# xiaoxubeii/kubernetes-schedule-simulator

Measured on AMD Instinct MI355X. Metric: pods scheduled/sec + node-evals/sec at 100k nodes, 1/2/4/8 MI355X, higher is better.
Workload: dtype int64; 1 GPU; C3: 100000 nodes, 1000000-pod queue, default predicates + LeastRequested(1) + BalancedResourceAllocation(1); nodes=100000, global_batch=35715, mode=persistent, blocks=256, parallelism=single-gpu

## Files before the change

include/ksim.h:

```cpp
#ifndef KSIM_H
#define KSIM_H

#include <stdint.h>

#ifdef __cplusplus
extern "C" {
#endif

#define KSIM_ABI_VERSION 7

#define KSIM_OK 0
#define KSIM_E_INVAL (-1)
#define KSIM_E_DEVICE (-2)
#define KSIM_E_NOMEM (-3)
#define KSIM_E_UNSUPPORTED (-4)
#define KSIM_E_STATE (-5)
#define KSIM_E_OVERFLOW (-6)
#define KSIM_E_NO_NODES (-7)

#define KSIM_MAX_SCALAR 8
#define KSIM_MAX_RCLASS 16
#define KSIM_MAX_WIDE 256
#define KSIM_NREASONS 32
#define KSIM_MAX_RANKS 8
// ... 351 lines not shown
  int64_t n_nodes;
  int32_t max_vols[3];
  int32_t zone_words;
  const uint32_t* key_filter;
  const int32_t* vc;
  const uint32_t* vc_filter;
  const ksim_vol_ref* refs;
  const uint32_t* zone_ok;
  const uint64_t* slots;
  const int32_t* slot_count;
} ksim_volume_tables;

int ksim_load_volumes(ksim_handle* h, const ksim_volume_tables* t);
int ksim_grow_volumes(ksim_handle* h, const ksim_volume_tables* t);
int ksim_read_volumes(ksim_handle* h, uint64_t* slots, int32_t* slot_count);

int ksim_read_nodes(ksim_handle* h, ksim_node_state* out);
int ksim_get_counter(ksim_handle* h, uint64_t* out);
int ksim_set_counter(ksim_handle* h, uint64_t value);

#define KSIM_FORM_FAST 1
#define KSIM_FORM_STREAM 2
#define KSIM_FORM_CACHED 4
#define KSIM_FORM_ROWS_SHIFT 8
int ksim_last_form(ksim_handle* h, int32_t* form);

int ksim_selftest(void);

#ifdef __cplusplus
}
#endif
#endif
```

kubernetes-schedule-simulator_amd/csrc/ksim_handle.h:

```cpp
#pragma once
#include <hip/hip_runtime.h>

#include <algorithm>
#include <atomic>
#include <array>
#include <cstdarg>
#include <cstdio>
#include <cstdlib>
#include <cstring>
#include <map>
#include <string>
#include <vector>

#include "ksim_common.h"
#include "ksim_pgen.h"
#include "ksim_sweep.h"
#include "ksim_tree.h"
#include "ksim_f64.h"

extern "C" hipError_t ksim_launch_scan(const KsimCtx* c, int npt, int collect, int grid, hipStream_t s);
extern "C" hipError_t ksim_launch_eval(const KsimCtx* c, int64_t pod, uint8_t* fit, uint32_t* reasons, int64_t* score,
                                       uint8_t* rcls, hipStream_t s);
extern "C" int ksim_scan_coresident(int npt, int collect, int grid);
extern "C" int ksim_one_npt(int64_t n);
// ... 4 lines not shown
extern "C" hipError_t ksim_launch_serve(const KsimCtx* c, const KsimServeArgs* a, int npt, int grid, int aux, hipStream_t s);
extern "C" hipError_t ksim_launch_ipa_pass(const KsimCtx* c, int npt, int grid, hipStream_t s);
extern "C" hipError_t ksim_launch_assume(const KsimCtx* c, int64_t pod, int64_t node, int32_t* status, hipStream_t s);
extern "C" hipError_t ksim_launch_persistent(const KsimCtx* c, const KsimCtx* cdev, uint64_t* granules, int grid,
                                             int lds_rows, hipStream_t s);
extern "C" int ksim_persistent_config(int64_t n, int* grid, int* lds_rows);
extern "C" size_t ksim_persistent_granule_bytes(int grid);
extern "C" hipError_t ksim_sweep_prepare(const int64_t* ac, const int64_t* am, int64_t n, double* dac, double* dam,
                                         double* yc, double* ym, hipStream_t st);
extern "C" hipError_t ksim_sweep_launch(const int64_t* rc0, const int64_t* rm0, const int64_t* zc0, const int64_t* zm0,
                                        const int32_t* c0, const ksim_pod* pods, void* fpods, const SwArgsWhy* args,
                                        int32_t n_scen, const uint32_t* absent, int32_t absent_words, hipEvent_t ev0,
                                        hipEvent_t ev1, hipStream_t st);
extern "C" hipError_t ksim_sweep_general_launch(const KsimCtx* hc, const SwgCols* cols, const SwgArgsPre* args,
                                                const SwgSpread* spr, const SwgAffinity* ipa, const SwgVolumes* vol,
                                                int32_t n_scen, const uint32_t* absent, int32_t absent_words,
                                                int32_t* err, hipEvent_t ev0, hipEvent_t ev1, hipStream_t st);
extern "C" int ksim_pfast_config(int64_t n, int max_grid, int stream, int* grid, int* lds_rows);
extern "C" hipError_t ksim_pstream_prepare(const KsimCtx* c, double* mirror, hipStream_t s);
extern "C" size_t ksim_pfast_granule_bytes(void);
extern "C" size_t ksim_shard_xchg_bytes(void);
extern "C" size_t ksim_shard_lx_offset(void);
extern "C" size_t ksim_pfast_cache_bytes(int lds_rows, int ncls);
extern "C" int ksim_pfast_rows_per_thread(int lds_rows, int stream);
extern "C" hipError_t ksim_launch_pfast(const KsimCtx* c, uint64_t* granules, int grid, int lds_rows, double* mirror,
                                        const KsimShard* sh, const int32_t* tcls, const KsimTreeClass* tclass, int ncls,
                                        hipStream_t s);
extern "C" hipError_t ksim_tree_build(const KsimCtx* c, const KsimTreeGeo* g, const KsimTreeClass* cls,
                                      const int32_t* tcls, int32_t* leaves, uint64_t* levels, int32_t* fitc,
                                      double* ty, const KsimTreeSweep* sw, hipStream_t s);
extern "C" hipError_t ksim_tree_build_absent(const KsimCtx* c, const KsimTreeGeo* g, const KsimTreeClass* cls,
                                             const int32_t* tcls, int32_t* leaves, uint64_t* levels, int32_t* fitc,
                                             double* ty, const KsimTreeSweep* sw, hipStream_t s);
extern "C" hipError_t ksim_tree_sweep_init(const KsimCtx* c, const KsimTreeSweep* sw, hipStream_t s);
extern "C" hipError_t ksim_tree_sweep_absent(const KsimCtx* c, const KsimTreeSweep* sw, const uint32_t* absent,
                                             int32_t words, hipStream_t s);
extern "C" hipError_t ksim_tree_launch(const KsimCtx* c, const KsimTreeGeo* g, const KsimTreeClass* cls,
                                       const int32_t* tcls, int32_t* leaves, uint64_t* levels, int32_t* fitc,
                                       double* ty, const KsimTreeSweep* sw, hipStream_t s);
struct KsimRelayout;
extern "C" hipError_t ksim_launch_relayout(const KsimRelayout* r, hipStream_t s);
extern "C" hipError_t ksim_launch_set_row(const KsimCtx* c, int64_t node, const uint64_t* pack, int32_t full,
                                          hipStream_t s);
extern "C" hipError_t ksim_launch_release(const KsimCtx* c, int64_t pod, int64_t node, hipStream_t s);
extern "C" hipError_t ksim_launch_undo(const KsimCtx* c, const KsimTentRec* t, hipStream_t s);
extern "C" hipError_t ksim_launch_remap_hosts(ksim_pod* pods, int64_t n_pods, int64_t idx, int32_t op, hipStream_t s);
extern "C" hipError_t ksim_launch_pod_k(ksim_pod* pods, int64_t n_pods, const KsimCtx* c, hipStream_t s);
extern "C" hipError_t ksim_launch_port_max(const int32_t* port_count, int64_t n, int32_t* out, hipStream_t s);

struct DevBuf {
// ... 257 lines not shown
```

kubernetes-schedule-simulator_amd/csrc/ksim_pfast.hip:

```cpp
#include <algorithm>

#include "ksim_decide.h"
#include "ksim_f64.h"
#include "ksim_fast.h"
#include "ksim_tree.h"
#include "ksim_wave.h"
#include "ksim_xchg.h"

using namespace kf64;

namespace {

#ifndef KSIM_PF_BS
#define KSIM_PF_BS 512
#endif
constexpr int BS = KSIM_PF_BS;
constexpr int NW = BS / 64;
constexpr int RW = NW - 1;
constexpr int RT = RW * 64;
constexpr int MAXB = 4;
constexpr int MAXG = 64 * MAXB;
constexpr int NSLOT = 4;
constexpr int FIXSTRIDE = 16;
constexpr int RING = 16;
constexpr int RING_FILL = 8;
constexpr uint64_t SPIN_LIMIT_TICKS = 200000000ull;
constexpr int ANSLOT = 8;
// ... 82 lines not shown
  int32_t rank, world;
  int64_t node_base;
  uint32_t xtag_base;
  uint64_t* xchg;
  uint64_t* peers[KSIM_MAX_RANKS];
  uint64_t start_ticks;
  double* mirror;
  const int32_t* tcls;
  const KsimTreeClass* tclass;
  int32_t ncls;
};

namespace {

struct FRows {
  double *ac, *am, *rc, *rm, *zc, *zm, *yc, *ym;
  int32_t *allowed, *count;
  uint32_t* fl;
  int32_t* ev;
  int32_t* ev2;
  uint32_t* rm2;
  uint32_t* rma;
  int16_t* cache;
};

constexpr int LDS_ROW_BYTES = 8 * 8 + 8 * 4;
constexpr int LDS_ROW_BYTES_STREAM = 7 * 4;

extern __shared__ __attribute__((aligned(16))) char kf_smem[];

template <bool STREAM>
__device__ __forceinline__ FRows carve(int rows, const PfArgs& a, int64_t lo) {
  FRows r;
  if (STREAM) {
    double* m = a.mirror + lo;
    const int64_t n = a.n;
    r.ac = m; r.am = m + n; r.rc = m + 2 * n; r.rm = m + 3 * n;
    r.zc = m + 4 * n; r.zm = m + 5 * n; r.yc = nullptr; r.ym = nullptr;
    r.allowed = const_cast<int32_t*>(a.allowed_pods) + lo;
    r.count = a.pod_count + lo;
    r.fl = const_cast<uint32_t*>(a.flags) + lo;
    int32_t* q = reinterpret_cast<int32_t*>(kf_smem);
    r.ev = q;
    r.ev2 = q + 2 * rows;
    r.rm2 = reinterpret_cast<uint32_t*>(q + 3 * rows);
    r.rma = r.rm2 + 2 * rows;
    r.cache = nullptr;
    return r;
  }
  double* d = reinterpret_cast<double*>(kf_smem);
  r.ac = d; r.am = d + rows; r.rc = d + 2 * rows; r.rm = d + 3 * rows;
  r.zc = d + 4 * rows; r.zm = d + 5 * rows; r.yc = d + 6 * rows; r.ym = d + 7 * rows;
  int32_t* q = reinterpret_cast<int32_t*>(d + 8 * rows);
  r.allowed = q; r.count = q + rows;
  r.fl = reinterpret_cast<uint32_t*>(q + 2 * rows);
  r.ev = q + 3 * rows;
  r.ev2 = q + 5 * rows;
  r.rm2 = reinterpret_cast<uint32_t*>(q + 6 * rows);
  r.cache = reinterpret_cast<int16_t*>(q + 8 * rows);
  return r;
}

typedef __attribute__((address_space(1))) const uint64_t cgu64;
typedef __attribute__((address_space(1))) const int32_t cgi32;
__device__ __forceinline__ double ld_l2(const double* p) {
  return __builtin_bit_cast(double, __hip_atomic_load((cgu64*)p, __ATOMIC_RELAXED, __HIP_MEMORY_SCOPE_AGENT));
}
__device__ __forceinline__ int32_t ld_l2(const int32_t* p) {
  return __hip_atomic_load((cgi32*)p, __ATOMIC_RELAXED, __HIP_MEMORY_SCOPE_AGENT);
}
__device__ __forceinline__ FRow load_frow_l2(const FRows& R, int32_t j) {
  FRow r;
  r.ac = ld_l2(R.ac + j); r.am = ld_l2(R.am + j); r.rc = ld_l2(R.rc + j); r.rm = ld_l2(R.rm + j);
  r.zc = ld_l2(R.zc + j); r.zm = ld_l2(R.zm + j);
  r.yc = r.ac != 0.0 ? 1.0 / r.ac : 0.0;
  r.ym = r.am != 0.0 ? 1.0 / r.am : 0.0;
  r.allowed = ld_l2(R.allowed + j); r.count = ld_l2(R.count + j);
  r.fl = (uint32_t)ld_l2(reinterpret_cast<const int32_t*>(R.fl) + j);
  return r;
}

template <bool STREAM>
__device__ __forceinline__ FRow load_frow(const FRows& R, int32_t j) {
  FRow r;
  r.ac = R.ac[j]; r.am = R.am[j]; r.rc = R.rc[j]; r.rm = R.rm[j]; r.zc = R.zc[j]; r.zm = R.zm[j];
  if (STREAM) {
    r.yc = r.ac != 0.0 ? 1.0 / r.ac : 0.0;
    r.ym = r.am != 0.0 ? 1.0 / r.am : 0.0;
  } else {
    r.yc = R.yc[j]; r.ym = R.ym[j];
  }
  r.allowed = R.allowed[j]; r.count = R.count[j]; r.fl = R.fl[j];
  return r;
}

struct Top2 {
  int32_t f, m1, c1, m2, c2;
};

}

template <int NPT, bool STREAM, bool CACHE>
__global__ __launch_bounds__(BS) void ksim_pfast_kernel(PfArgs a) {
  static_assert(!(STREAM && CACHE), "the cached form keeps the rows in LDS");
  __shared__ int32_t s_wst[2][RW][5];
  __shared__ uint64_t s_bm[2][NPT][RW];
  __shared__ int32_t s_wg[2][5];
  __shared__ int32_t s_fix[2][2];
  __shared__ int32_t s_hist[KSIM_NREASONS];
  __shared__ int32_t s_mode[2], s_own[2];
  __shared__ int32_t s_arr;
  __shared__ int32_t s_prow[2];
  __shared__ double s_pdel[2][4];
  __shared__ double s_pval[4];
  __shared__ int32_t s_pcnt;
  __shared__ __attribute__((aligned(16))) ksim_pod s_pod[RING];
  __shared__ int32_t s_pcls[CACHE ? RING : 1];
  __shared__ KsimTreeClass s_tcl[CACHE ? KSIM_TREE_MAX_CLASSES : 1];
#ifdef KSIM_STAMPS
  uint64_t st_acc[16] = {};
#endif

  const int tid = threadIdx.x, lane = tid & 63, wv = tid >> 6;
  const int rt = tid - 64;
  const int G = gridDim.x;
  const int me = blockIdx.x;
  const int64_t chunk = a.chunk;
  const int64_t lo = (int64_t)me * chunk;
// ... 28 lines not shown
    if (p < a.end) reinterpret_cast<uint4*>(&s_pod[p % RING])[lane % 8] = v;
    if (CACHE && lane < RING_FILL && p0 + lane < a.end) s_pcls[(p0 + lane) % RING] = cl;
  };
  uint4 ring_next = make_uint4(0, 0, 0, 0);
  int32_t ring_next_cl = 0;
  if (wv == 1) {
    uint4 v;
    int32_t cl = 0;
    ring_load(a.first, v, cl);
    ring_load(a.first + RING_FILL, ring_next, ring_next_cl);
    ring_store(a.first, v, cl);
  }
  if (CACHE)
    for (int k = tid; k < a.ncls; k += BS) s_tcl[k] = a.tclass[k];
  if (tid == 0) { s_fix[a.first & 1][0] = -1; s_arr = 0; s_prow[0] = s_prow[1] = -1; }
  uint64_t counter = *a.counter;
  __syncthreads();
  auto cls_fpod = [&](int k) -> FPod {
    const KsimTreeClass& t = s_tcl[k];
    return FPod{t.rq_c, t.rq_m, t.nz_c, t.nz_m, 0.0, 0.0, t.anyreq, t.be};
  };
  if (CACHE) {
    const int tot = a.ncls * nrows;
    for (int idx = tid; idx < tot; idx += BS) {
      const int k = idx / nrows, j = idx - k * nrows;
      uint32_t rm;
      R.cache[k * chunk + j] = (int16_t)feval(EC, cls_fpod(k), load_frow<false>(R, j), rm);
    }
    __syncthreads();
  }

  auto ptag = [&](int64_t p) -> uint64_t { return (uint64_t)((p - a.first + 1) & 0xFF); };
  auto wave_stats = [&](const int32_t (&e)[NPT], int buf, int w) {
    int32_t v = -1, nf = 0;
#pragma unroll
    for (int k = 0; k < NPT; ++k) {
      nf += __popcll(__ballot(e[k] >= 0));
      v = e[k] > v ? e[k] : v;
    }
    const int32_t m1 = ksimw::max_i32(v);
    int32_t v2 = -1;
#pragma unroll
    for (int k = 0; k < NPT; ++k) v2 = (e[k] < m1 && e[k] > v2) ? e[k] : v2;
    const int32_t m2 = ksimw::max_i32(v2);
    int32_t c1 = 0, c2 = 0;
#pragma unroll
    for (int k = 0; k < NPT; ++k) {
      const uint64_t bm = m1 < 0 ? 0ull : __ballot(e[k] == m1);
      c1 += __popcll(bm);
      c2 += m2 < 0 ? 0 : __popcll(__ballot(e[k] == m2));
// ... 11 lines not shown
    old = __builtin_amdgcn_readfirstlane(old);
    if ((old + 1) % RW == 0) {
      __builtin_amdgcn_fence(__ATOMIC_ACQUIRE, "workgroup", "local");
      const bool in = lane < RW;
      const int w = in ? lane : 0;
      const int32_t f = in ? s_wst[buf][w][0] : 0;
      const int32_t a1 = s_wst[buf][w][1], n1 = in ? s_wst[buf][w][2] : 0;
      const int32_t a2 = s_wst[buf][w][3], n2 = in ? s_wst[buf][w][4] : 0;
      Top2 t;
      t.f = ksimw::sum_i32(f);
      t.m1 = ksimw::max_i32(n1 ? a1 : -1);
      t.c1 = ksimw::sum_i32((n1 && a1 == t.m1) ? n1 : 0);
      t.m2 = ksimw::max_i32(n1 && a1 < t.m1 ? a1 : (n2 ? a2 : -1));
      t.c2 = ksimw::sum_i32(((n1 && a1 == t.m2) ? n1 : 0) + ((n2 && a2 == t.m2) ? n2 : 0));
      if (t.m2 < 0) t.c2 = 0;
      if (lane == 0) {
        s_wg[buf][0] = t.f; s_wg[buf][1] = t.m1; s_wg[buf][2] = t.c1; s_wg[buf][3] = t.m2; s_wg[buf][4] = t.c2;
        if (NR == 1) ksimx::store_agent((gu64*)spec_at(granules, (int)(p % NSLOT), me), gpack(ptag(p), t.f, t.c1, t.m1));
      }
      if (NR > 1 && lane < NR)
        ksimx::store_agent((gu64*)spec_at(granules + lane * REP_STRIDE, (int)(p % NSLOT), me), gpack(ptag(p), t.f, t.c1, t.m1));
    }
  };
  struct Segs {
    uint64_t m;
    int32_t cnt, base, total;
  };
  auto seg_prepare = [&](int buf) -> Segs {
    constexpr int S = NPT * RW;
    const int32_t M = s_wg[buf][1];
    Segs sg;
    sg.m = 0;
    if (lane < S) {
      const int k = NPT - 1 - lane / RW, w = RW - 1 - lane % RW;
      sg.m = (M >= 0 && s_wst[buf][w][1] == M) ? s_bm[buf][k][w] : 0ull;
    }
    sg.cnt = __popcll(sg.m);
    const int32_t incl = ksimw::prefix_incl_i32(sg.cnt);
    sg.base = incl - sg.cnt;
    sg.total = __builtin_amdgcn_readlane(incl, 63);
    return sg;
  };
  auto seg_select = [&](const Segs& sg, int32_t rank) -> int32_t {
    const uint64_t hs = __ballot(sg.cnt != 0 && rank >= sg.base && rank < sg.base + sg.cnt);
    if (rank >= sg.total || !hs) return -1;
    const int t = __builtin_ctzll(hs);
    const uint64_t ms = ((uint64_t)(uint32_t)__builtin_amdgcn_readlane((int32_t)(sg.m >> 32), t) << 32) |
                        (uint64_t)(uint32_t)__builtin_amdgcn_readlane((int32_t)sg.m, t);
    const int32_t r = rank - __builtin_amdgcn_readlane(sg.base, t);
    const uint64_t hb = __ballot(((ms >> lane) & 1ull) && __popcll(ms >> lane) - 1 == r);
    if (!hb) return -1;
    const int k = NPT - 1 - t / RW, w = RW - 1 - t % RW;
    return k * RT + w * 64 + __builtin_ctzll(hb);
  };

  auto build_top_list = [&](int buf) {
    constexpr int S = NPT * RW;
    const int32_t M = s_wg[buf][1];
// ... 15 lines not shown
      if ((ms >> lane) & 1ull) top_list[b0 + __popcll(ms >> lane) - 1] = k * RT + w * 64 + lane;
    }
  };

  uint32_t A_rm[STREAM ? 1 : NPT], B_rm[STREAM ? 1 : NPT];
  if (wv > 0) {
    const FPod P0 = load_fpod(s_pod[a.first % RING]);
    int32_t e[NPT];
    int32_t* ev = R.ev + (a.first & 1) * chunk;
#pragma unroll
    for (int k = 0; k < NPT; ++k) {
      const int32_t j = k * RT + rt;
      e[k] = -1;
      uint32_t& am = A_rm[STREAM ? 0 : k];
      am = 0;
      if (CACHE) {
        if (j < nrows) e[k] = R.cache[s_pcls[a.first % RING] * chunk + j];
      } else if (j < nrows) {
        e[k] = feval(EC, P0, load_frow<STREAM>(R, j), am);
        if (STREAM) R.rma[(a.first & 1) * chunk + j] = am;
        ev[j] = e[k];
      }
    }
    wave_stats(e, (int)(a.first & 1), wv);
    arrive_publish(a.first, (int)(a.first & 1));
  }
  int X = -1;
  int64_t stop_at = a.end;
  lds_barrier();
#ifdef KSIM_STAMPS
  uint64_t t_prev = __builtin_amdgcn_s_memtime();
  uint64_t tb_prev = t_prev, bw_busy = 0, bw_wait = 0;
#endif

  int64_t last = a.first;
  for (int64_t pod = a.first; pod < a.end; ++pod) {
    last = pod;
    const bool has_next = pod + 1 < a.end;
    const int pb = (int)(pod & 1);
    const int nb = (int)((pod + 1) & 1);
    int32_t jsel = -1;
    uint64_t stopbit = 0;
    FRow jrow;
    int32_t e_new = -1;
    uint32_t m_new = 0;
#ifdef KSIM_STAMPS
    uint64_t o_prev = 0;
#endif

    if (wv == 0) {
      Segs sg{};
      if (STREAM) build_top_list(pb);
      else sg = seg_prepare(pb);
      STAMP(1);
      const uint64_t tag = ptag(pod);
      const int slot = (int)(pod % NSLOT);
      uint64_t g[MAXB], fx = 0;
      bool ok = false;
      const uint64_t t0 = __builtin_amdgcn_s_memrealtime();
      for (;;) {
#pragma unroll
        for (int j = 0; j < MAXB; ++j) g[j] = ksimx::load_agent((gu64*)my_rep + slot * MAXG + j * 64 + lane);
        fx = ksimx::load_agent((gu64*)fix_at(my_rep, slot));
        bool mine = X < 0 || gtag(fx) == tag;
#pragma unroll
        for (int j = 0; j < MAXB; ++j) {
          const int b = lane * MAXB + j;
          mine &= (b >= G) || b == X || gtag(g[j]) == tag;
        }
        if (__all(mine)) {
          ok = true;
#pragma unroll
          for (int j = 0; j < MAXB; ++j) g[j] = (lane * MAXB + j == X) ? fx : g[j];
          break;
        }
        if (__builtin_amdgcn_s_memrealtime() - t0 > SPIN_LIMIT_TICKS) break;
// ... 69 lines not shown
      }
      const uint64_t hb = __ballot(hit);
      const int src = __builtin_ffsll((long long)hb) - 1;
      const int blk = hb ? __builtin_amdgcn_readlane(found, src) : -1;
      const int rank = hb ? __builtin_amdgcn_readlane((int32_t)rr, src) : 0;
      int mode;
      if (!ok) mode = -1;
      else if (stop_any) mode = -2;
      else if (F == 0) mode = 0;
      else if (hb) mode = blk >= 0 ? 2 : -1;
      else mode = a.world > 1 ? 3 : -1;
      if (mode >= 2 && F > 1) counter += 1;
      if (lane == 0 && mode == -1) atomicOr(a.err, ok ? 2 : 4);
      STAMP(3);
#ifdef KSIM_STAMPS
      o_prev = __builtin_amdgcn_s_memtime();
#endif
      if (mode == 2 && blk == me) {
        jsel = STREAM ? (rank < s_wg[pb][2] ? top_list[rank] : -1) : seg_select(sg, rank);
        if (jsel < 0 || jsel >= nrows) {
          jsel = -1;
          mode = -1;
          if (lane == 0) atomicOr(a.err, 2);
        } else if (!STREAM) {
          const ksim_pod& Pp = s_pod[pod % RING];
          stopbit = (R.rc[jsel] + (double)Pp.add_cpu >= EXACT_LIM || R.rm[jsel] + (double)Pp.add_mem >= EXACT_LIM ||
                     R.zc[jsel] + (double)Pp.nz_cpu >= EXACT_LIM || R.zm[jsel] + (double)Pp.nz_mem >= EXACT_LIM)
                        ? (1ull << 55)
                        : 0ull;
        } else if (has_next) {
          jrow = load_frow_l2(R, jsel);
          if (jsel != s_prow[nb]) {
            const FRow r2 = plus(jrow, load_fpod(s_pod[pod % RING]));
            e_new = feval(EC, load_fpod(s_pod[(pod + 1) % RING]), r2, m_new);
            stopbit = (r2.rc >= EXACT_LIM || r2.rm >= EXACT_LIM || r2.zc >= EXACT_LIM || r2.zm >= EXACT_LIM) ? (1ull << 55) : 0ull;
          }
        }
        OSTAMP(22);
      }
      if ((mode == 0 || mode == 3) && me == 0 && lane == 0) a.out_node[pod] = mode == 0 ? -1 : -2;
      if (lane == 0) {
        s_mode[pb] = mode;
        s_own[pb] = jsel;
        if (STREAM) {
          s_prow[pb] = jsel;
          if (jsel >= 0) {
// ... 25 lines not shown
      if (has_next) {
      const bool refill = wv == 1 && ((pod - a.first) % RING_FILL) == 0;
      if (refill) ring_store(pod + RING_FILL, ring_next, ring_next_cl);
      uint4 rv;
      int32_t rcl = 0;
      if (refill) ring_load(pod + 2 * RING_FILL, rv, rcl);
#ifdef KSIM_STAMPS
      const uint64_t te0 = __builtin_amdgcn_s_memtime();
#endif
      PROBE(4);
      const FPod P = load_fpod(s_pod[pod % RING]);
      const FPod Q = load_fpod(s_pod[(pod + 1) % RING]);
#ifdef KSIM_STAMPS
      uint64_t tw = __builtin_amdgcn_s_memtime();
      if (tid == 64) st_acc[8] += tw - te0;
#define WSTAMP(k) do { const uint64_t t_ = __builtin_amdgcn_s_memtime(); if (tid == 64) st_acc[k] += t_ - tw; tw = t_; } while (0)
#else
#define WSTAMP(k) do { } while (0)
#endif
      int32_t e[NPT];
      FRow rk[STREAM ? 1 : NPT];
      int32_t* evn = R.ev + nb * chunk;
      if (CACHE) {
        const int16_t* c1 = R.cache + s_pcls[(pod + 1) % RING] * chunk;
#pragma unroll
        for (int k = 0; k < NPT; ++k) {
          const int32_t j = k * RT + rt;
          e[k] = j < nrows ? (int32_t)c1[j] : -1;
        }
        WSTAMP(9);
        wave_stats(e, nb, wv);
        WSTAMP(10);
        arrive_publish(pod + 1, nb);
        const int32_t M0 = s_wg[pb][1];
        const int16_t* c0 = R.cache + s_pcls[pod % RING] * chunk;
#pragma unroll
        for (int k = 0; k < NPT; ++k) {
          const int32_t j = k * RT + rt;
          if (M0 >= 0 && j < nrows && (int32_t)c0[j] == M0) {
            uint32_t m2;
            R.ev2[j] = feval(EC, Q, plus(load_frow<false>(R, j), P), m2);
            R.rm2[j] = m2;
          }
        }
      } else {
#pragma unroll
      for (int k = 0; k < NPT; ++k) {
        const int32_t j = k * RT + rt;
        e[k] = -1;
        uint32_t& bm = B_rm[STREAM ? 0 : k];
        bm = 0;
        if (j < nrows) {
          FRow r = load_frow<STREAM>(R, j);
          if (STREAM && j == prow) apply_commit(r, j);
          e[k] = feval(EC, Q, r, bm);
          evn[j] = e[k];
// ... 41 lines not shown
      tb_prev = tb1;
    }
#endif
    STAMP(7);
    const int mode = s_mode[pb];
    if (mode < 0) {
      if (mode == -2) stop_at = pod;
      break;
    }
    const int32_t own = s_own[pb];

    if (own >= 0) {
      if (wv == 0) {
        OSTAMP(17);
        if (has_next) {
          if (STREAM && jsel == s_prow[nb]) {
            FRow r = jrow;
            r.rc = s_pval[0]; r.rm = s_pval[1]; r.zc = s_pval[2]; r.zm = s_pval[3]; r.count = s_pcnt;
            const FRow r2 = plus(r, load_fpod(s_pod[pod % RING]));
            e_new = feval(EC, load_fpod(s_pod[(pod + 1) % RING]), r2, m_new);
            stopbit = (r2.rc >= EXACT_LIM || r2.rm >= EXACT_LIM || r2.zc >= EXACT_LIM || r2.zm >= EXACT_LIM) ? (1ull << 55) : 0ull;
          }
          if (!STREAM) { e_new = R.ev2[jsel]; m_new = R.rm2[jsel]; }
          const int32_t e_old = CACHE ? (int32_t)R.cache[s_pcls[(pod + 1) % RING] * chunk + jsel] : R.ev[nb * chunk + jsel];
          const int32_t f0 = s_wg[nb][0], m1 = s_wg[nb][1], c1 = s_wg[nb][2], m2 = s_wg[nb][3], c2 = s_wg[nb][4];
          const bool rem = e_old >= 0, add = e_new >= 0;
          const int32_t c1a = c1 - ((rem && e_old == m1) ? 1 : 0);
          const int32_t mb = c1a ? m1 : (c2 ? m2 : -1), cb = c1a ? c1a : c2;
          const bool up = add && (cb == 0 || e_new > mb), eq = add && !up && e_new == mb;
          const int32_t M = up ? e_new : mb, Cn = up ? 1 : cb + (eq ? 1 : 0);
          const int32_t Ff = f0 - (rem ? 1 : 0) + (add ? 1 : 0);
          PROBE(2);
          if (NR > 1 && lane < NR)
            ksimx::store_agent((gu64*)fix_at(granules + lane * REP_STRIDE, (int)((pod + 1) % NSLOT)),
                          gpack(ptag(pod + 1), Ff, Cn, Cn ? M : -1) | stopbit);
          if (lane == 0) {
            if (NR == 1)
              ksimx::store_agent((gu64*)fix_at(granules, (int)((pod + 1) % NSLOT)), gpack(ptag(pod + 1), Ff, Cn, Cn ? M : -1) | stopbit);
            s_wg[nb][0] = Ff; s_wg[nb][1] = Cn ? M : -1; s_wg[nb][2] = Cn;
          }
        }
        OSTAMP(18);
        if (CACHE) {
          const FRow r2 = plus(load_frow<false>(R, jsel), load_fpod(s_pod[pod % RING]));
          if (lane < a.ncls) {
            uint32_t rm;
            R.cache[lane * chunk + jsel] = (int16_t)feval(EC, cls_fpod(lane), r2, rm);
          }
        }
        if (lane == 0) {
          if (!STREAM) {
            const ksim_pod& Pp = s_pod[pod % RING];
            R.rc[jsel] += (double)Pp.add_cpu; R.rm[jsel] += (double)Pp.add_mem;
            R.zc[jsel] += (double)Pp.nz_cpu; R.zm[jsel] += (double)Pp.nz_mem;
            R.count[jsel] += 1;
          }
          if (stopbit) atomicOr(a.err, 8);
          a.out_node[pod] = (int32_t)(a.node_base + lo + jsel);
          if (has_next) {
            R.ev[nb * chunk + jsel] = e_new;
            s_fix[nb][0] = jsel;
            s_fix[nb][1] = (int32_t)m_new;
          } else {
            s_fix[nb][0] = -1;
          }
        }
      }
      lds_barrier();
      if (wv == 0 && has_next) {
        const int w = 1 + (jsel % RT) / 64;
        int32_t e[NPT];
#pragma unroll
        for (int k = 0; k < NPT; ++k) {
          const int32_t j = k * RT + (w - 1) * 64 + lane;
          e[k] = j < nrows ? (CACHE ? (int32_t)R.cache[s_pcls[(pod + 1) % RING] * chunk + j] : R.ev[nb * chunk + j]) : -1;
        }
        wave_stats(e, nb, w);
        OSTAMP(19);
#ifdef KSIM_STAMPS
        if (lane == 0) atomicAdd((unsigned long long*)&a.dbg[21], 1ull);
#endif
      }
    } else if (wv == 0 && lane == 0) {
      s_fix[nb][0] = -1;
    }

    if (mode == 0 && a.collect && a.out_reasons) {
      if (tid < KSIM_NREASONS) s_hist[tid] = 0;
      lds_barrier();
      if (wv > 0) {
        const int32_t fr = s_fix[pb][0];
        const uint32_t fmk = (uint32_t)s_fix[pb][1];
// ... 96 lines not shown
    m[i] = dac;
    m[n + i] = dam;
    m[2 * n + i] = (double)rc[i];
    m[3 * n + i] = (double)rm[i];
    m[4 * n + i] = (double)zc[i];
    m[5 * n + i] = (double)zm[i];
  }
}

extern "C" hipError_t ksim_pstream_prepare(const KsimCtx* c, double* mirror, hipStream_t s) {
  const int pg = (int)std::min<int64_t>((c->n + 255) / 256, 4096);
  hipLaunchKernelGGL(ksim_pstream_prepare_kernel, dim3(pg), dim3(256), 0, s, c->alloc_cpu, c->alloc_mem,
                     (const int64_t*)c->req_cpu, (const int64_t*)c->req_mem, (const int64_t*)c->nz_cpu,
                     (const int64_t*)c->nz_mem, c->n, mirror);
  return hipGetLastError();
}

extern "C" size_t ksim_pfast_cache_bytes(int lds_rows, int ncls) {
  if (ncls <= 0 || ncls > KSIM_TREE_MAX_CLASSES || lds_rows <= 0) return 0;
  const size_t b = ((size_t)ncls * lds_rows * 2 + 15) & ~(size_t)15;
  return (size_t)lds_rows * LDS_ROW_BYTES + b <= (size_t)PF_LDS_BUDGET ? b : 0;
}

extern "C" int ksim_pfast_rows_per_thread(int lds_rows, int stream) {
  return lds_rows <= RT ? 1 : lds_rows <= 2 * RT ? 2 : (lds_rows <= 4 * RT || !stream) ? 4 : 9;
}

extern "C" hipError_t ksim_launch_pfast(const KsimCtx* c, uint64_t* granules, int grid, int lds_rows, double* mirror,
                                        const KsimShard* sh, const int32_t* tcls, const KsimTreeClass* tclass, int ncls,
                                        hipStream_t s) {
  PfArgs a;
  a.tcls = tcls; a.tclass = tclass; a.ncls = ncls;
  a.rank = sh->rank; a.world = sh->world; a.node_base = sh->node_base; a.xtag_base = sh->xtag_base;
  a.xchg = sh->xchg;
  for (int r = 0; r < KSIM_MAX_RANKS; ++r) a.peers[r] = sh->peers[r];
  a.start_ticks = sh->start_ticks > SPIN_LIMIT_TICKS ? sh->start_ticks : SPIN_LIMIT_TICKS;
  a.n = c->n; a.chunk = c->chunk; a.first = c->first; a.end = c->end;
  a.alloc_cpu = c->alloc_cpu; a.alloc_mem = c->alloc_mem; a.allowed_pods = c->allowed_pods; a.flags = c->flags;
  a.req_cpu = c->req_cpu; a.req_mem = c->req_mem; a.nz_cpu = c->nz_cpu; a.nz_mem = c->nz_mem;
  a.pod_count = c->pod_count; a.pods = c->pods; a.counter = c->counter; a.cursor = c->cursor;
  a.out_node = c->out_node; a.out_reasons = c->out_reasons; a.err = c->err; a.dbg = c->dbg; a.granules = granules;
  a.preds = c->preds; a.no_prio = c->no_prio; a.collect = c->collect;
  a.wl = (int32_t)c->w[KSIM_W_LEAST_REQUESTED]; a.wm = (int32_t)c->w[KSIM_W_MOST_REQUESTED];
  a.wb = (int32_t)c->w[KSIM_W_BALANCED];
  a.mirror = mirror;
#define KSIM_PFC(R, S, C, L)                                                           \
  do {                                                                                 \
    hipError_t e_ = ksim_check_coresident(ksim_pfast_kernel<R, S, C>, grid, BS, L);    \
    if (e_ != hipSuccess) return e_;                                                   \
    hipLaunchKernelGGL((ksim_pfast_kernel<R, S, C>), dim3(grid), dim3(BS), L, s, a);   \
  } while (0)
#define KSIM_PF(R, S, L) KSIM_PFC(R, S, false, L)
  if (mirror) {
    const size_t lds = (size_t)lds_rows * LDS_ROW_BYTES_STREAM;
    if (lds_rows <= RT) KSIM_PF(1, true, lds);
    else if (lds_rows <= 2 * RT) KSIM_PF(2, true, lds);
    else if (lds_rows <= 4 * RT) KSIM_PF(4, true, lds);
    else KSIM_PF(9, true, lds);
    return hipGetLastError();
  }
  const size_t cb = ncls > 0 ? ksim_pfast_cache_bytes(lds_rows, ncls) : 0;
  if (ncls > 0 && !cb) return hipErrorInvalidValue;
  const size_t lds = (size_t)lds_rows * LDS_ROW_BYTES + cb;
  if (cb) {
    if (lds_rows <= RT) KSIM_PFC(1, false, true, lds);
    else if (lds_rows <= 2 * RT) KSIM_PFC(2, false, true, lds);
    else KSIM_PFC(4, false, true, lds);
    return hipGetLastError();
  }
  if (lds_rows <= RT) KSIM_PF(1, false, lds);
  else if (lds_rows <= 2 * RT) KSIM_PF(2, false, lds);
  else KSIM_PF(4, false, lds);
#undef KSIM_PF
#undef KSIM_PFC
  return hipGetLastError();
}
```

kubernetes-schedule-simulator_amd/csrc/ksim_runtime.cpp:

```cpp
#include "ksim_handle.h"

namespace {
thread_local std::string g_err;
}

int ksim_fail(ksim_handle* h, int code, const char* fmt, ...) {
  char buf[512];
  va_list ap;
  va_start(ap, fmt);
  vsnprintf(buf, sizeof buf, fmt, ap);
  va_end(ap);
  if (h) h->err = buf;
  g_err = buf;
  return code;
}

extern "C" {

int ksim_abi_version(void) { return KSIM_ABI_VERSION; }

const char* ksim_last_error(const ksim_handle* h) { return h ? h->err.c_str() : g_err.c_str(); }

int ksim_create(const ksim_config* cfg, ksim_handle** out) {
  if (!cfg || !out) return ksim_fail(nullptr, KSIM_E_INVAL, "ksim_create: null argument");
// ... 695 lines not shown

static int run_persistent_mode(ksim_handle* h, int64_t first, int64_t count, ksim_stats* st);

static int run_pfast_mode(ksim_handle* h, int64_t first, int64_t count, int grid, int lds_rows, bool stream,
                          ksim_stats* st) {
  KsimCtx& c = h->ctx;
  if (stream) {
    if (!h->mirror) {
      int rc = dev_alloc(h, &h->mirror, (size_t)6 * c.n);
      if (rc) return rc;
    }
    hipError_t e = ksim_pstream_prepare(&c, h->mirror, ksim_stream(h));
    if (e != hipSuccess) return ksim_fail(h, KSIM_E_DEVICE, "stream prepare: %s", hipGetErrorString(e));
  }
  const size_t gb = ksim_pfast_granule_bytes();
  if (h->gran_bytes < gb) {
    int rc = dev_alloc(h, &h->granules, gb / sizeof(uint64_t));
    if (rc) return rc;
    h->gran_bytes = gb;
  }
  c.first = first;
  c.end = first + count;
  c.chunk = (c.n + grid - 1) / grid;
  int ncls = 0;
  if (!stream && !getenv("KSIM_NO_PCACHE") && h->n_tcls > 0 && h->tcls && h->tclass) {
    int64_t sw = 0;
    for (int k : {KSIM_W_LEAST_REQUESTED, KSIM_W_MOST_REQUESTED, KSIM_W_BALANCED}) sw += c.no_prio ? 0 : c.w[k] * 10;
    if (sw < 32767 && ksim_pfast_cache_bytes(lds_rows, h->n_tcls)) ncls = h->n_tcls;
  }
  h->last_pfast_cache = ncls > 0;
  h->last_form = KSIM_FORM_FAST | (stream ? KSIM_FORM_STREAM : 0) | (ncls > 0 ? KSIM_FORM_CACHED : 0) |
                 (ksim_pfast_rows_per_thread(lds_rows, stream ? 1 : 0) << KSIM_FORM_ROWS_SHIFT);
  HIPCHK(h, hipMemsetAsync(h->granules, 0, gb, ksim_stream(h)));
  HIPCHK(h, hipEventRecord(h->ev0, ksim_stream(h)));
  hipError_t e = ksim_launch_pfast(&c, h->granules, grid, lds_rows, stream ? h->mirror : nullptr, &h->shard, h->tcls,
                                   h->tclass, ncls, ksim_stream(h));
  if (e == hipErrorCooperativeLaunchTooLarge) {
    h->last_form = 0;
    if (h->cfg.mode != KSIM_MODE_PERSISTENT && h->shard.world == 1) {
      h->pfast_off = true;
      return run_persistent_mode(h, first, count, st);
    }
    return ksim_fail(h, KSIM_E_UNSUPPORTED, "persistent launch: %d workgroups cannot be co-resident on this device", grid);
  }
  if (e != hipSuccess) return ksim_fail(h, KSIM_E_DEVICE, "persistent launch: %s", hipGetErrorString(e));
  HIPCHK(h, hipEventRecord(h->ev1, ksim_stream(h)));
  HIPCHK(h, hipEventSynchronize(h->ev1));
  float ms = 0.f;
  HIPCHK(h, hipEventElapsedTime(&ms, h->ev0, h->ev1));
#ifdef KSIM_STAMPS
  {
    uint64_t d[64];
    HIPCHK(h, hipMemcpy(d, c.dbg, sizeof d, hipMemcpyDeviceToHost));
    HIPCHK(h, hipMemset(c.dbg, 0, sizeof d));
    const double nf = (double)(d[21] ? d[21] : 1);
    {
    fprintf(stderr, "[ksim stamps] pfast workgroup 0, per wave (0 = control) cycles/pod between main barriers busy/wait:");
    for (int w = 0; w < 8; ++w) fprintf(stderr, " %d:%.0f/%.0f", w, d[32 + w] / (double)count, d[40 + w] / (double)count);
    fprintf(stderr, "\n");
// ... 717 lines not shown
```

kubernetes-schedule-simulator_amd/ksim/abi.py:

```python
from __future__ import annotations

import ctypes as C
import os

import numpy as np

PKG_DIR = os.path.dirname(os.path.dirname(os.path.abspath(__file__)))
LIB_PATH = os.environ.get("KSIM_LIB") or os.path.join(PKG_DIR, "lib", "libksim.so")

KSIM_OK = 0
E_INVAL, E_DEVICE, E_NOMEM, E_UNSUPPORTED, E_STATE, E_OVERFLOW, E_NO_NODES = -1, -2, -3, -4, -5, -6, -7
ABI_VERSION = 7
MAX_SCALAR = 8
MAX_RCLASS = 16
MAX_WIDE = 256
SWEEP_GENERAL_MAX_NODES = 38400
SWEEP_SPREAD_MAX_ZONES = 512
NREASONS = 32

P_CHECK_NODE_CONDITION = 1 << 0
P_CHECK_NODE_UNSCHEDULABLE = 1 << 1
P_GENERAL = 1 << 2
P_HOSTNAME = 1 << 3
P_HOST_PORTS = 1 << 4
# ... 150 lines not shown
class NodeState(C.Structure):
    _fields_ = [("req_cpu", _i64p), ("req_mem", _i64p), ("req_gpu", _i64p), ("req_eph", _i64p),
                ("nz_cpu", _i64p), ("nz_mem", _i64p), ("pod_count", _i32p), ("req_scalar", _i64p),
                ("ports", _u64p), ("port_count", _i32p)]


POD_DTYPE = np.dtype([("req_cpu", "<i8"), ("req_mem", "<i8"), ("req_gpu", "<i8"), ("req_eph", "<i8"),
                      ("add_cpu", "<i8"), ("add_mem", "<i8"), ("add_gpu", "<i8"), ("add_eph", "<i8"),
                      ("nz_cpu", "<i8"), ("nz_mem", "<i8"), ("cls", "<i4"), ("host", "<i4"), ("flags", "<u4"),
                      ("port_off", "<i4"), ("port_cnt", "<i4"), ("scalar_off", "<i4"), ("scalar_cnt", "<i4"),
                      ("aff_ident", "<i4"), ("aff_class", "<i4"), ("vol_class", "<i4"),
                      ("reserved", "<i4", (2,))])
SCALAR_DTYPE = np.dtype([("col", "<i4"), ("pad", "<i4"), ("req", "<i8"), ("add", "<i8")])
assert POD_DTYPE.itemsize == C.sizeof(Pod) == 128
assert SCALAR_DTYPE.itemsize == C.sizeof(ScalarReq)

EXPORTS = ["ksim_abi_version", "ksim_last_error", "ksim_create", "ksim_destroy", "ksim_load_nodes",
           "ksim_load_classes", "ksim_load_pods", "ksim_schedule", "ksim_evaluate", "ksim_assume",
           "ksim_read_nodes", "ksim_get_counter", "ksim_set_counter", "ksim_selftest", "ksim_sweep",
           "ksim_shard_setup", "ksim_shard_export", "ksim_shard_connect", "ksim_shard_connect_local",
           "ksim_schedule_one", "ksim_pod_add", "ksim_pod_remove", "ksim_node_add", "ksim_node_update",
           "ksim_node_remove", "ksim_node_count", "ksim_append_pods", "ksim_load_affinity", "ksim_load_volumes",
           "ksim_read_volumes", "ksim_grow_volumes", "ksim_sweep_nodes", "ksim_last_form"]
FORM_FAST, FORM_STREAM, FORM_CACHED, FORM_ROWS_SHIFT = 1, 2, 4, 8
IPC_HANDLE_BYTES = 64
MAX_RANKS = 8


class KsimError(RuntimeError):
    def __init__(self, code, msg):
        super().__init__("ksim error %d: %s" % (code, msg))
        self.code = code


class KsimUnsupported(KsimError):
    pass


class NoNodesAvailable(KsimError):
    """core.ErrNoNodesAvailable (generic_scheduler.go:64): "no nodes available to schedule pods"."""


_lib = None


def lib():
    global _lib
# ... 107 lines not shown
```

Measured before the change: 452,900 pods/s.

## Track per-class score histograms in LDS to get top score without wave scans

Adds a per-class 64-bucket histogram of cached node scores in LDS, kept up to date incrementally when a node is bound. The top score, its count and the feasible count for the next pod are then read from the histogram with a ballot instead of rescanning every cached row with wave_stats. The per-wave best-row bitmaps are patched for a single bit when the top score is unchanged and rebuilt only when it moves. This costs extra LDS and atomics at cache build, and applies only when the summed priority weights keep scores at 63 or below.

```diff
diff --git a/include/ksim.h b/include/ksim.h
--- a/include/ksim.h
+++ b/include/ksim.h
@@ -397,6 +397,7 @@
 #define KSIM_FORM_FAST 1
 #define KSIM_FORM_STREAM 2
 #define KSIM_FORM_CACHED 4
+#define KSIM_FORM_HIST 8
 #define KSIM_FORM_ROWS_SHIFT 8
 int ksim_last_form(ksim_handle* h, int32_t* form);
 
diff --git a/kubernetes-schedule-simulator_amd/csrc/ksim_handle.h b/kubernetes-schedule-simulator_amd/csrc/ksim_handle.h
--- a/kubernetes-schedule-simulator_amd/csrc/ksim_handle.h
+++ b/kubernetes-schedule-simulator_amd/csrc/ksim_handle.h
@@ -50,10 +50,11 @@
 extern "C" size_t ksim_shard_xchg_bytes(void);
 extern "C" size_t ksim_shard_lx_offset(void);
 extern "C" size_t ksim_pfast_cache_bytes(int lds_rows, int ncls);
+extern "C" size_t ksim_pfast_hist_bytes(int lds_rows, int ncls);
 extern "C" int ksim_pfast_rows_per_thread(int lds_rows, int stream);
 extern "C" hipError_t ksim_launch_pfast(const KsimCtx* c, uint64_t* granules, int grid, int lds_rows, double* mirror,
                                         const KsimShard* sh, const int32_t* tcls, const KsimTreeClass* tclass, int ncls,
-                                        hipStream_t s);
+                                        int hist, hipStream_t s);
 extern "C" hipError_t ksim_tree_build(const KsimCtx* c, const KsimTreeGeo* g, const KsimTreeClass* cls,
                                       const int32_t* tcls, int32_t* leaves, uint64_t* levels, int32_t* fitc,
                                       double* ty, const KsimTreeSweep* sw, hipStream_t s);
diff --git a/kubernetes-schedule-simulator_amd/csrc/ksim_pfast.hip b/kubernetes-schedule-simulator_amd/csrc/ksim_pfast.hip
--- a/kubernetes-schedule-simulator_amd/csrc/ksim_pfast.hip
+++ b/kubernetes-schedule-simulator_amd/csrc/ksim_pfast.hip
@@ -3,6 +3,7 @@
 #include "ksim_decide.h"
 #include "ksim_f64.h"
 #include "ksim_fast.h"
+#include "ksim_phist.h"
 #include "ksim_tree.h"
 #include "ksim_wave.h"
 #include "ksim_xchg.h"
@@ -131,6 +132,7 @@
   uint32_t* rm2;
   uint32_t* rma;
   int16_t* cache;
+  uint16_t* hist;
 };
 
 constexpr int LDS_ROW_BYTES = 8 * 8 + 8 * 4;
@@ -155,6 +157,7 @@
     r.rm2 = reinterpret_cast<uint32_t*>(q + 3 * rows);
     r.rma = r.rm2 + 2 * rows;
     r.cache = nullptr;
+    r.hist = nullptr;
     return r;
   }
   double* d = reinterpret_cast<double*>(kf_smem);
@@ -167,6 +170,7 @@
   r.ev2 = q + 5 * rows;
   r.rm2 = reinterpret_cast<uint32_t*>(q + 6 * rows);
   r.cache = reinterpret_cast<int16_t*>(q + 8 * rows);
+  r.hist = reinterpret_cast<uint16_t*>(reinterpret_cast<char*>(r.cache) + (((size_t)a.ncls * rows * 2 + 15) & ~(size_t)15));
   return r;
 }
 
@@ -209,10 +213,11 @@
 
 }
 
-template <int NPT, bool STREAM, bool CACHE>
+template <int NPT, bool STREAM, bool CACHE, bool HIST = false>
 __global__ __launch_bounds__(BS) void ksim_pfast_kernel(PfArgs a) {
   static_assert(!(STREAM && CACHE), "the cached form keeps the rows in LDS");
-  __shared__ int32_t s_wst[2][RW][5];
+  static_assert(!HIST || CACHE, "the histograms count the cached evaluations");
+  __shared__ int32_t s_wst[HIST ? 1 : 2][HIST ? 1 : RW][5];
   __shared__ uint64_t s_bm[2][NPT][RW];
   __shared__ int32_t s_wg[2][5];
   __shared__ int32_t s_fix[2][2];
@@ -287,10 +292,17 @@
   };
   if (CACHE) {
     const int tot = a.ncls * nrows;
+    uint32_t* const hw = reinterpret_cast<uint32_t*>(R.hist);
+    if (HIST) {
+      for (int i = tid; i < a.ncls * (KSIM_PHIST_BUCKETS / 2); i += BS) hw[i] = 0;
+      __syncthreads();
+    }
     for (int idx = tid; idx < tot; idx += BS) {
       const int k = idx / nrows, j = idx - k * nrows;
       uint32_t rm;
-      R.cache[k * chunk + j] = (int16_t)feval(EC, cls_fpod(k), load_frow<false>(R, j), rm);
+      const int32_t ev = feval(EC, cls_fpod(k), load_frow<false>(R, j), rm);
+      R.cache[k * chunk + j] = (int16_t)ev;
+      if (HIST && ev >= 0) atomicAdd(&hw[k * (KSIM_PHIST_BUCKETS / 2) + khist::word(ev)], khist::unit(ev));
     }
     __syncthreads();
   }
@@ -348,6 +360,28 @@
         ksimx::store_agent((gu64*)spec_at(granules + lane * REP_STRIDE, (int)(p % NSLOT), me), gpack(ptag(p), t.f, t.c1, t.m1));
     }
   };
+  auto hist_publish = [&](int64_t p, int buf) {
+    const int cls = s_pcls[p % RING];
+    const int32_t h = R.hist[cls * KSIM_PHIST_BUCKETS + lane];
+    const int32_t M = khist::top(__ballot(h != 0));
+    if (wv == 1) {
+      const int32_t F = ksimw::sum_i32(h);
+      const int32_t C = __builtin_amdgcn_readlane(h, M < 0 ? 0 : M);
+      if (lane == 0) {
+        s_wg[buf][0] = F; s_wg[buf][1] = M; s_wg[buf][2] = C;
+        if (NR == 1) ksimx::store_agent((gu64*)spec_at(granules, (int)(p % NSLOT), me), gpack(ptag(p), F, C, M));
+      }
+      if (NR > 1 && lane < NR)
+        ksimx::store_agent((gu64*)spec_at(granules + lane * REP_STRIDE, (int)(p % NSLOT), me), gpack(ptag(p), F, C, M));
+    }
+    const int16_t* c1 = R.cache + cls * chunk;
+#pragma unroll
+    for (int k = 0; k < NPT; ++k) {
+      const int32_t j = k * RT + rt;
+      const uint64_t bm = __ballot(M >= 0 && j < nrows && (int32_t)c1[j] == M);
+      if (lane == 0) s_bm[buf][k][wv - 1] = bm;
+    }
+  };
   struct Segs {
     uint64_t m;
     int32_t cnt, base, total;
@@ -359,7 +393,8 @@
     sg.m = 0;
     if (lane < S) {
       const int k = NPT - 1 - lane / RW, w = RW - 1 - lane % RW;
-      sg.m = (M >= 0 && s_wst[buf][w][1] == M) ? s_bm[buf][k][w] : 0ull;
+      if constexpr (HIST) sg.m = M >= 0 ? s_bm[buf][k][w] : 0ull;
+      else sg.m = (M >= 0 && s_wst[buf][w][1] == M) ? s_bm[buf][k][w] : 0ull;
     }
     sg.cnt = __popcll(sg.m);
     const int32_t incl = ksimw::prefix_incl_i32(sg.cnt);
@@ -421,8 +456,12 @@
         ev[j] = e[k];
       }
     }
-    wave_stats(e, (int)(a.first & 1), wv);
-    arrive_publish(a.first, (int)(a.first & 1));
+    if constexpr (HIST) {
+      hist_publish(a.first, (int)(a.first & 1));
+    } else {
+      wave_stats(e, (int)(a.first & 1), wv);
+      arrive_publish(a.first, (int)(a.first & 1));
+    }
   }
   int X = -1;
   int64_t stop_at = a.end;
@@ -443,6 +482,10 @@
     FRow jrow;
     int32_t e_new = -1;
     uint32_t m_new = 0;
+    int32_t hM_old = -1, hM_new = -1;
+    int32_t hcls = 0, hrow = 0, hF0 = 0;
+    int32_t he_old = -1;
+    double hdel[4] = {0.0, 0.0, 0.0, 0.0};
 #ifdef KSIM_STAMPS
     uint64_t o_prev = 0;
 #endif
@@ -451,6 +494,16 @@
       Segs sg{};
       if (STREAM) build_top_list(pb);
       else sg = seg_prepare(pb);
+      if constexpr (HIST) {
+        if (has_next) {
+          hcls = s_pcls[(pod + 1) % RING];
+          hrow = R.hist[hcls * KSIM_PHIST_BUCKETS + lane];
+          hF0 = ksimw::sum_i32(hrow);
+          hM_old = khist::top(__ballot(hrow != 0));
+        }
+        const ksim_pod& Pp = s_pod[pod % RING];
+        hdel[0] = (double)Pp.add_cpu; hdel[1] = (double)Pp.add_mem; hdel[2] = (double)Pp.nz_cpu; hdel[3] = (double)Pp.nz_mem;
+      }
       STAMP(1);
       const uint64_t tag = ptag(pod);
       const int slot = (int)(pod % NSLOT);
@@ -566,6 +619,10 @@
           jsel = -1;
           mode = -1;
           if (lane == 0) atomicOr(a.err, 2);
+        } else if (HIST) {
+          const double s0 = R.rc[jsel] + hdel[0], s1 = R.rm[jsel] + hdel[1], s2 = R.zc[jsel] + hdel[2], s3 = R.zm[jsel] + hdel[3];
+          if (has_next) he_old = (int32_t)R.cache[hcls * chunk + jsel];
+          stopbit = ((s0 >= EXACT_LIM) | (s1 >= EXACT_LIM) | (s2 >= EXACT_LIM) | (s3 >= EXACT_LIM)) ? (1ull << 55) : 0ull;
         } else if (!STREAM) {
           const ksim_pod& Pp = s_pod[pod % RING];
           stopbit = (R.rc[jsel] + (double)Pp.add_cpu >= EXACT_LIM || R.rm[jsel] + (double)Pp.add_mem >= EXACT_LIM ||
@@ -637,16 +694,22 @@
       FRow rk[STREAM ? 1 : NPT];
       int32_t* evn = R.ev + nb * chunk;
       if (CACHE) {
-        const int16_t* c1 = R.cache + s_pcls[(pod + 1) % RING] * chunk;
-#pragma unroll
-        for (int k = 0; k < NPT; ++k) {
-          const int32_t j = k * RT + rt;
-          e[k] = j < nrows ? (int32_t)c1[j] : -1;
-        }
-        WSTAMP(9);
-        wave_stats(e, nb, wv);
-        WSTAMP(10);
-        arrive_publish(pod + 1, nb);
+        if constexpr (HIST) {
+          WSTAMP(9);
+          hist_publish(pod + 1, nb);
+          WSTAMP(10);
+        } else {
+          const int16_t* c1 = R.cache + s_pcls[(pod + 1) % RING] * chunk;
+#pragma unroll
+          for (int k = 0; k < NPT; ++k) {
+            const int32_t j = k * RT + rt;
+            e[k] = j < nrows ? (int32_t)c1[j] : -1;
+          }
+          WSTAMP(9);
+          wave_stats(e, nb, wv);
+          WSTAMP(10);
+          arrive_publish(pod + 1, nb);
+        }
         const int32_t M0 = s_wg[pb][1];
         const int16_t* c0 = R.cache + s_pcls[pod % RING] * chunk;
 #pragma unroll
@@ -734,14 +797,29 @@
             stopbit = (r2.rc >= EXACT_LIM || r2.rm >= EXACT_LIM || r2.zc >= EXACT_LIM || r2.zm >= EXACT_LIM) ? (1ull << 55) : 0ull;
           }
           if (!STREAM) { e_new = R.ev2[jsel]; m_new = R.rm2[jsel]; }
-          const int32_t e_old = CACHE ? (int32_t)R.cache[s_pcls[(pod + 1) % RING] * chunk + jsel] : R.ev[nb * chunk + jsel];
-          const int32_t f0 = s_wg[nb][0], m1 = s_wg[nb][1], c1 = s_wg[nb][2], m2 = s_wg[nb][3], c2 = s_wg[nb][4];
+          int32_t e_old, f0, m1 = -1, c1 = 0, m2 = -1, c2 = 0;
+          if constexpr (HIST) {
+            e_old = he_old;
+            f0 = hF0;
+          } else {
+            e_old = CACHE ? (int32_t)R.cache[s_pcls[(pod + 1) % RING] * chunk + jsel] : R.ev[nb * chunk + jsel];
+            f0 = s_wg[nb][0]; m1 = s_wg[nb][1]; c1 = s_wg[nb][2]; m2 = s_wg[nb][3]; c2 = s_wg[nb][4];
+          }
           const bool rem = e_old >= 0, add = e_new >= 0;
-          const int32_t c1a = c1 - ((rem && e_old == m1) ? 1 : 0);
-          const int32_t mb = c1a ? m1 : (c2 ? m2 : -1), cb = c1a ? c1a : c2;
-          const bool up = add && (cb == 0 || e_new > mb), eq = add && !up && e_new == mb;
-          const int32_t M = up ? e_new : mb, Cn = up ? 1 : cb + (eq ? 1 : 0);
           const int32_t Ff = f0 - (rem ? 1 : 0) + (add ? 1 : 0);
+          int32_t M, Cn;
+          if constexpr (HIST) {
+            const int32_t h = khist::adjusted(hrow, lane, e_old, e_new);
+            M = khist::top(__ballot(h != 0));
+            Cn = __builtin_amdgcn_readlane(h, M < 0 ? 0 : M);
+            hM_new = M;
+          } else {
+            const int32_t c1a = c1 - ((rem && e_old == m1) ? 1 : 0);
+            const int32_t mb = c1a ? m1 : (c2 ? m2 : -1), cb = c1a ? c1a : c2;
+            const bool up = add && (cb == 0 || e_new > mb), eq = add && !up && e_new == mb;
+            M = up ? e_new : mb;
+            Cn = up ? 1 : cb + (eq ? 1 : 0);
+          }
           PROBE(2);
           if (NR > 1 && lane < NR)
             ksimx::store_agent((gu64*)fix_at(granules + lane * REP_STRIDE, (int)((pod + 1) % NSLOT)),
@@ -757,7 +835,9 @@
           const FRow r2 = plus(load_frow<false>(R, jsel), load_fpod(s_pod[pod % RING]));
           if (lane < a.ncls) {
             uint32_t rm;
-            R.cache[lane * chunk + jsel] = (int16_t)feval(EC, cls_fpod(lane), r2, rm);
+            const int32_t en = feval(EC, cls_fpod(lane), r2, rm);
+            if constexpr (HIST) khist::move(R.hist + lane * KSIM_PHIST_BUCKETS, (int32_t)R.cache[lane * chunk + jsel], en);
+            R.cache[lane * chunk + jsel] = (int16_t)en;
           }
         }
         if (lane == 0) {
@@ -779,7 +859,27 @@
         }
       }
       lds_barrier();
-      if (wv == 0 && has_next) {
+      if (HIST && wv == 0 && has_next) {
+        if (hM_new == hM_old) {
+          if (lane == 0 && hM_new >= 0) {
+            uint64_t& m = s_bm[nb][jsel / RT][(jsel % RT) / 64];
+            const uint64_t bit = 1ull << (jsel & 63);
+            m = e_new == hM_new ? (m | bit) : (m & ~bit);
+          }
+        } else {
+          const int16_t* c1 = R.cache + s_pcls[(pod + 1) % RING] * chunk;
+          for (int sgi = 0; sgi < NPT * RW; ++sgi) {
+            const int32_t j = sgi * 64 + lane;
+            const uint64_t bm = __ballot(hM_new >= 0 && j < nrows && (int32_t)c1[j] == hM_new);
+            if (lane == 0) s_bm[nb][sgi / RW][sgi % RW] = bm;
+          }
+        }
+        OSTAMP(19);
+#ifdef KSIM_STAMPS
+        if (lane == 0) atomicAdd((unsigned long long*)&a.dbg[21], 1ull);
+#endif
+      }
+      if (!HIST && wv == 0 && has_next) {
         const int w = 1 + (jsel % RT) / 64;
         int32_t e[NPT];
 #pragma unroll
@@ -922,13 +1022,20 @@
   return (size_t)lds_rows * LDS_ROW_BYTES + b <= (size_t)PF_LDS_BUDGET ? b : 0;
 }
 
+extern "C" size_t ksim_pfast_hist_bytes(int lds_rows, int ncls) {
+  const size_t cb = ksim_pfast_cache_bytes(lds_rows, ncls);
+  if (!cb) return 0;
+  const size_t hb = (size_t)ncls * KSIM_PHIST_BUCKETS * sizeof(uint16_t);
+  return (size_t)lds_rows * LDS_ROW_BYTES + cb + hb <= (size_t)PF_LDS_BUDGET ? hb : 0;
+}
+
 extern "C" int ksim_pfast_rows_per_thread(int lds_rows, int stream) {
   return lds_rows <= RT ? 1 : lds_rows <= 2 * RT ? 2 : (lds_rows <= 4 * RT || !stream) ? 4 : 9;
 }
 
 extern "C" hipError_t ksim_launch_pfast(const KsimCtx* c, uint64_t* granules, int grid, int lds_rows, double* mirror,
                                         const KsimShard* sh, const int32_t* tcls, const KsimTreeClass* tclass, int ncls,
-                                        hipStream_t s) {
+                                        int hist, hipStream_t s) {
   PfArgs a;
   a.tcls = tcls; a.tclass = tclass; a.ncls = ncls;
   a.rank = sh->rank; a.world = sh->world; a.node_base = sh->node_base; a.xtag_base = sh->xtag_base;
@@ -961,7 +1068,22 @@
   }
   const size_t cb = ncls > 0 ? ksim_pfast_cache_bytes(lds_rows, ncls) : 0;
   if (ncls > 0 && !cb) return hipErrorInvalidValue;
-  const size_t lds = (size_t)lds_rows * LDS_ROW_BYTES + cb;
+  const size_t hb = hist ? ksim_pfast_hist_bytes(lds_rows, ncls) : 0;
+  if (hist && !hb) return hipErrorInvalidValue;
+  const size_t lds = (size_t)lds_rows * LDS_ROW_BYTES + cb + hb;
+  if (hb) {
+#define KSIM_PFH(R, L)                                                                         \
+  do {                                                                                         \
+    hipError_t e_ = ksim_check_coresident(ksim_pfast_kernel<R, false, true, true>, grid, BS, L); \
+    if (e_ != hipSuccess) return e_;                                                           \
+    hipLaunchKernelGGL((ksim_pfast_kernel<R, false, true, true>), dim3(grid), dim3(BS), L, s, a); \
+  } while (0)
+    if (lds_rows <= RT) KSIM_PFH(1, lds);
+    else if (lds_rows <= 2 * RT) KSIM_PFH(2, lds);
+    else KSIM_PFH(4, lds);
+#undef KSIM_PFH
+    return hipGetLastError();
+  }
   if (cb) {
     if (lds_rows <= RT) KSIM_PFC(1, false, true, lds);
     else if (lds_rows <= 2 * RT) KSIM_PFC(2, false, true, lds);
diff --git a/kubernetes-schedule-simulator_amd/csrc/ksim_phist.h b/kubernetes-schedule-simulator_amd/csrc/ksim_phist.h
--- /dev/null
+++ b/kubernetes-schedule-simulator_amd/csrc/ksim_phist.h
@@ -0,0 +1,50 @@
+#pragma once
+#include <stdint.h>
+
+#ifdef __HIPCC__
+#include <hip/hip_runtime.h>
+#define KSIM_PHIST_FN __host__ __device__ inline
+#else
+#define KSIM_PHIST_FN inline
+#endif
+
+#define KSIM_PHIST_BUCKETS 64
+
+namespace khist {
+
+KSIM_PHIST_FN int word(int s) { return s >> 1; }
+KSIM_PHIST_FN uint32_t unit(int s) { return 1u << ((s & 1) * 16); }
+
+KSIM_PHIST_FN void build(uint32_t* row, const int16_t* col, int n) {
+  for (int s = 0; s < KSIM_PHIST_BUCKETS / 2; ++s) row[s] = 0;
+  for (int j = 0; j < n; ++j)
+    if (col[j] >= 0) row[word(col[j])] += unit(col[j]);
+}
+
+KSIM_PHIST_FN void move(uint16_t* row, int e_old, int e_new) {
+  if (e_old == e_new) return;
+  if (e_old >= 0) row[e_old] -= 1;
+  if (e_new >= 0) row[e_new] += 1;
+}
+
+KSIM_PHIST_FN int32_t adjusted(int32_t h, int s, int e_old, int e_new) {
+  return h - (s == e_old ? 1 : 0) + (s == e_new ? 1 : 0);
+}
+
+KSIM_PHIST_FN int top(uint64_t nonempty) { return nonempty ? 63 - __builtin_clzll(nonempty) : -1; }
+
+KSIM_PHIST_FN void stats(const uint16_t* row, int e_old, int e_new, int32_t* F, int32_t* M, int32_t* C) {
+  uint64_t ne = 0;
+  int32_t f = 0;
+  for (int s = 0; s < KSIM_PHIST_BUCKETS; ++s) {
+    const int32_t h = adjusted(row[s], s, e_old, e_new);
+    f += h;
+    ne |= (uint64_t)(h != 0) << s;
+  }
+  const int m = top(ne);
+  *F = f;
+  *M = m;
+  *C = m < 0 ? 0 : adjusted(row[m], m, e_old, e_new);
+}
+
+}
diff --git a/kubernetes-schedule-simulator_amd/csrc/ksim_runtime.cpp b/kubernetes-schedule-simulator_amd/csrc/ksim_runtime.cpp
--- a/kubernetes-schedule-simulator_amd/csrc/ksim_runtime.cpp
+++ b/kubernetes-schedule-simulator_amd/csrc/ksim_runtime.cpp
@@ -741,19 +741,21 @@
   c.first = first;
   c.end = first + count;
   c.chunk = (c.n + grid - 1) / grid;
-  int ncls = 0;
+  int ncls = 0, hist = 0;
   if (!stream && !getenv("KSIM_NO_PCACHE") && h->n_tcls > 0 && h->tcls && h->tclass) {
     int64_t sw = 0;
     for (int k : {KSIM_W_LEAST_REQUESTED, KSIM_W_MOST_REQUESTED, KSIM_W_BALANCED}) sw += c.no_prio ? 0 : c.w[k] * 10;
     if (sw < 32767 && ksim_pfast_cache_bytes(lds_rows, h->n_tcls)) ncls = h->n_tcls;
+    if (ncls > 0 && sw <= 63 && !getenv("KSIM_NO_PHIST") && ksim_pfast_hist_bytes(lds_rows, ncls)) hist = 1;
   }
   h->last_pfast_cache = ncls > 0;
   h->last_form = KSIM_FORM_FAST | (stream ? KSIM_FORM_STREAM : 0) | (ncls > 0 ? KSIM_FORM_CACHED : 0) |
+                 (hist ? KSIM_FORM_HIST : 0) |
                  (ksim_pfast_rows_per_thread(lds_rows, stream ? 1 : 0) << KSIM_FORM_ROWS_SHIFT);
   HIPCHK(h, hipMemsetAsync(h->granules, 0, gb, ksim_stream(h)));
   HIPCHK(h, hipEventRecord(h->ev0, ksim_stream(h)));
   hipError_t e = ksim_launch_pfast(&c, h->granules, grid, lds_rows, stream ? h->mirror : nullptr, &h->shard, h->tcls,
-                                   h->tclass, ncls, ksim_stream(h));
+                                   h->tclass, ncls, hist, ksim_stream(h));
   if (e == hipErrorCooperativeLaunchTooLarge) {
     h->last_form = 0;
     if (h->cfg.mode != KSIM_MODE_PERSISTENT && h->shard.world == 1) {
diff --git a/kubernetes-schedule-simulator_amd/ksim/abi.py b/kubernetes-schedule-simulator_amd/ksim/abi.py
--- a/kubernetes-schedule-simulator_amd/ksim/abi.py
+++ b/kubernetes-schedule-simulator_amd/ksim/abi.py
@@ -196,7 +196,7 @@
            "ksim_schedule_one", "ksim_pod_add", "ksim_pod_remove", "ksim_node_add", "ksim_node_update",
            "ksim_node_remove", "ksim_node_count", "ksim_append_pods", "ksim_load_affinity", "ksim_load_volumes",
            "ksim_read_volumes", "ksim_grow_volumes", "ksim_sweep_nodes", "ksim_last_form"]
-FORM_FAST, FORM_STREAM, FORM_CACHED, FORM_ROWS_SHIFT = 1, 2, 4, 8
+FORM_FAST, FORM_STREAM, FORM_CACHED, FORM_HIST, FORM_ROWS_SHIFT = 1, 2, 4, 8, 8
 IPC_HANDLE_BYTES = 64
 MAX_RANKS = 8
 
```

Measured after the change: 483,800 pods/s (median of 6 runs). 1.07x the previous value.
